# rwl/blu

Measured on AMD Instinct MI355X. Metric: factorize nnz/s + achieved HBM GB/s, 100k x 100k 10-nnz/col basis, higher is better.
Workload: dtype f64

## Files before the change

blu_amd/csrc/blu_dev.h:

```cpp
#pragma once
#include <hip/hip_runtime.h>
#include <stdint.h>
#include <hip/hip_cooperative_groups.h>
#include <rocprim/warp/warp_reduce.hpp>
#include <rocprim/warp/warp_scan.hpp>

#define BLU_WAVE 64

#ifndef BLU_DYN_SHARED
#define BLU_DYN_SHARED(T, name, bytes) extern __shared__ __attribute__((aligned(16))) T name[]
#endif
#ifdef BLU_PROFILE_FILLS
#define FILL_STAMP_BEGIN() long long fill_t0_ = (long long)__builtin_amdgcn_s_memtime()
#define FILL_STAMP(S, k)                                                 \
    do {                                                                 \
        if (threadIdx.x == 0) {                                          \
            const long long t_ = (long long)__builtin_amdgcn_s_memtime(); \
            (S)->prof[k] += t_ - fill_t0_;                               \
            fill_t0_ = t_;                                               \
        }                                                                \
    } while (0)
#else
#define FILL_STAMP_BEGIN() \
    do {                   \
// ... 33 lines not shown
    int bump_size;
    int cused, rused;
    int lused, uused;
    int need;
    int l_nz, u_nz;
    int fill_paths;
    long long matrix_nz;
    long long bump_nz;
    long long nsearch_pivot;
    long long factor_flops;
    long long nexpand;
    long long ngarbage;
    long long d3_hits;
    long long npivot_kind[6];
    long long nfast[4];
    long long nrun[2];
    double min_pivot, max_pivot;
    double onenorm, infnorm;
    double norm_l, norm_u, normest_l_inv, normest_u_inv, condest_l, condest_u, residual_test;
    long long prof[48];
    long long prof2[8];
};

#define DEVLU_SCALARS(X)                                                                               \
    X(int, m)                                                                                          \
    X(int, nzbias)                                                                      \
    X(int, maxsearch)                                                                                  \
    X(int, pad)                                                                                        \
    X(int, search_rows)                                                                                \
    X(int, no_fast)                    \
    X(int, skip_stats)              \
    X(double, droptol)                                                                                 \
    X(double, abstol)                                                                                  \
    X(double, reltol)                                                                                  \
    X(double, stretch)                                                                                 \
    X(long long, b_i_len)                                                                              \
// ... 515 lines not shown
```

blu_amd/csrc/blu_hip.hip:

```cpp
#include <hip/hip_runtime.h>

#include <algorithm>
#include <cmath>
#include <cstdio>
#include <cstdlib>
#include <cstring>
#include <string>
#include <vector>

#include "../../include/blu_hip.h"
#include "blu_dev.h"
#include "k_finish.hip"
#define BLU_NS pv_single
#define BLU_CFG_WAVE 0
#include "k_pivot.hip"
#undef BLU_NS
#undef BLU_CFG_WAVE
#define BLU_NS pv_wave
#define BLU_CFG_WAVE 1
#include "k_pivot.hip"
#undef BLU_NS
#undef BLU_CFG_WAVE
#define BLU_NS pv_wave2
#define BLU_CFG_WAVE 2
// ... 475 lines not shown
    case 51: return (double)s.npivot_kind[0];
    case 52: return (double)s.npivot_kind[1];
    case 53: return (double)s.npivot_kind[2];
    case 54: return (double)s.npivot_kind[3];
    case 55: return (double)s.npivot_kind[4];
    case 56: return (double)s.npivot_kind[5];
    case 110: case 111: case 116: case 117: return (double)s.nfast[key < 116 ? key - 110 : key - 114];
    case 112: return (double)s.cused;
    case 113: return (double)s.rused;
    case 114: return (double)h->D.carena_cap;
    case 115: return (double)h->D.lcap;
    case 120: return (double)h->last_pivot_regs;
    case 118: return (double)h->last_pivot_kernel;
    case 119: return (double)s.fill_paths;
    case 121: case 122: return (double)s.nrun[key - 121];
    case 131: case 132: case 133: case 134: case 135: case 136: case 137: case 138: return (double)s.prof2[key - 131];
    case 57: return (double)s.err_line;
    case 58: return (double)s.status;
    case 60: case 61: case 62: case 63: case 64: case 65: case 66: case 67: case 68: case 69: case 70: case 71: case 72: case 73: case 74: case 75:
    case 76: case 77: case 78: case 79: case 80: case 81: case 82: case 83:
    case 84: case 85: case 86: case 87: case 88: case 89: case 90: case 91:
    case 92: case 93: case 94: case 95: case 96: case 97: case 98: case 99: case 100: case 101: case 102: case 103: case 104: case 105: case 106: case 107:
        return (double)s.prof[key - 60];
    default: return NAN;
    }
}

extern "C" const char *blu_hip_last_error(const blu_hip *h) { return h ? h->err.c_str() : "null handle"; }
extern "C" const char *blu_hip_version(void)
{
#if defined(BLU_EWCHECK)
// ... 632 lines not shown
```

blu_amd/csrc/k_pivot.hip:

```cpp
#include "blu_dev.h"

namespace BLU_NS {

__shared__ int g_pivot_err;
__shared__ int g_pivot_err_line;
#undef DEV_CHECK
#define DEV_CHECK(S, cond)                               \
    do {                                                 \
        if (!(cond)) {                                   \
            set_error((S), ST_ERROR, __LINE__);          \
            g_pivot_err = 1;                             \
        }                                                \
    } while (0)

#if BLU_CFG_WAVE
#include "k_pivot_wave_types.h"
#else
#include "k_pivot_fast_types.h"
#endif

#ifdef BLU_PROFILE
__shared__ long long g_pstamp[56];
#define PROF_STAMP(k)                                                      \
    do {                                                                   \
// ... 14 lines not shown
#define PROF_WAIT() \
    do {            \
    } while (0)
#endif

struct alignas(16) Sm {
    Fast fa;
    struct alignas(16) {
        int pr, pc, exit_code, head_exit;
    };
    struct alignas(16) {
        int nzc, nzr, pcb, prb;
    };
#ifdef BLU_PROFILE
    long long prof[48];
    long long prof2[8];
#else
    long long prof[1];
#endif
#if !BLU_CFG_WAVE
    Fast fb;
    struct alignas(16) {
        int nx_pr, nx_pc, nx_nzr, nx_where;
    };
    int nx_prb, nx_pcb, nx_nsr;
    int mg;
    long long nrun[2];
#endif
    int rank, rankdef, min_colnz, min_rownz;
    int cused, rused, lused, uused;
    int need;
    int flag_small;
    int other_row, where, ncancel, nfill;
    int stop_at, need_search;
    double pivot, other_value;
    long long nsearch, flops, nexpand, d3;
    long long kinds[6];
    long long nfast[4];
    int sh[40];
    long long shl[20];
#if BLU_CFG_WAVE
    unsigned long long wmax[BLU_CFG_WAVE];
// ... 1057 lines not shown
        sm->uused = S->uused;
        sm->pr = S->pivot_row;
        sm->pc = S->pivot_col;
        sm->exit_code = 0;
        sm->need = 0;
        sm->nsearch = 0;
        sm->flops = 0;
        sm->nexpand = 0;
        sm->d3 = 0;
        sm->stop_at = stop_at;
        sm->fa.kind = 0;
        sm->fa.ewValid = 0;
        sm->fa.spOk = 0;
        for (int k = 0; k < 6; k++) sm->kinds[k] = 0;
        sm->mg = 0;
        sm->nrun[0] = sm->nrun[1] = 0;
#ifdef BLU_PROFILE
        for (int k = 0; k < 48; k++) sm->prof[k] = 0;
        for (int k = 0; k < 8; k++) sm->prof2[k] = 0;
        for (int k = 0; k < 56; k++) g_pstamp[k] = 0;
#endif
    }
    for (int k = tid; k < (int)blockDim.x; k += blockDim.x) sm->swork[k] = 0.0;
    if (tid < 16) sm->wmax[tid] = 0ull;
    for (int k = tid; k < 2 * KGMAX; k += blockDim.x) sm->fa.kg[0][k] = 0ull;
    if (tid == 0) {
        g_pivot_err = 0;
        g_pivot_err_line = 0;
    }
    mc_reset(D, mc, tid, (int)blockDim.x);
    __syncthreads();

#ifdef BLU_PROFILE
#define PROF_ADD(k, a, b)                                                                                           \
    do {                                                                                                            \
        const long long d_ = g_pstamp[a] - g_pstamp[b];                                                             \
        if (g_pstamp[b] >= g_pstamp[0] && d_ >= 0 && d_ < (1LL << 28)) sm->prof[k] += d_;                            \
    } while (0)
#define PROF_ADD2(k, a, b)                                                                                          \
    do {                                                                                                            \
        const long long d_ = g_pstamp[a] - g_pstamp[b];                                                             \
        if (g_pstamp[b] >= g_pstamp[0] && d_ >= 0 && d_ < (1LL << 28)) sm->prof2[k] += d_;                           \
    } while (0)
    auto prof_account = [&](int kind_done) {
        {
            const int kk = kind_done == 1 ? 1 : (kind_done == 2 ? 2 : 3);
            PROF_ADD(0, 1, 0);
            PROF_ADD(kk, 2, 1);
            sm->prof[3 + kk] += 1;
            if (kk == 1) {
                PROF_ADD(7, 3, 1);
                PROF_ADD(22, 6, 3);
                PROF_ADD(23, 24, 3);
                PROF_ADD(24, 25, 3);
                PROF_ADD(25, 26, 25);
                PROF_ADD(26, 27, 26);
                PROF_ADD(27, 28, 27);
                PROF_ADD(30, 30, 27);
                PROF_ADD(31, 31, 30);
                PROF_ADD(28, 29, 28);
                PROF_ADD(29, 2, 29);
                sm->prof[32] += sm->nzr - 1;
                sm->prof[33] += sm->nzc - 1;
                PROF_ADD(34, 33, 1);
                PROF_ADD(35, 34, 33);
                PROF_ADD(36, 35, 34);
                PROF_ADD(37, 36, 35);
                PROF_ADD(38, 37, 36);
                PROF_ADD(39, 38, 37);
                PROF_ADD(40, 3, 38);
                if (g_pstamp[44] > g_pstamp[1]) {
                    PROF_ADD(41, 41, 1);
                    PROF_ADD(42, 42, 41);
                    PROF_ADD(43, 43, 42);
                    PROF_ADD(44, 44, 43);
                    sm->prof[45] += 1;
                }
            }
            if (kk == 2) {
                PROF_ADD2(0, 1, 0);
                PROF_ADD2(1, 49, 48);
                PROF_ADD2(2, 50, 48);
                PROF_ADD2(3, 51, 48);
                PROF_ADD2(4, 2, 48);
                PROF_ADD2(5, 48, 1);
            }
            if (kk != 3) {
                PROF_ADD(8, 8, 0);
                PROF_ADD(9, 9, 8);
                PROF_ADD(10, 10, 9);
                PROF_ADD(11, 11, 10);
// ... 62 lines not shown
        if (pr < 0) {
            __syncthreads();
            if (tid == 0) {
                list_remove1(D.cflink, D.cblink, pc);
                mc->dirty = 1;
                sm->pc = -1;
                sm->rankdef++;
                sm->kinds[5]++;
            }
            __syncthreads();
            continue;
        }

        if (dA.z) break;
        PROF_STAMP(1);
        const int nz_col = dB.x;
        int nz_row = dB.y;
        const int kind = dC.x;
        bool ok = true;
        if (kind == 1) fast_small(D, sm, mc, pr, pc, nz_col, nz_row, ew_mcb, ew_fb);
        else if (kind == 2) {
            Fast *cs = &sm->fa;
            int wq = dC.y;
            for (;;) {
                fast_scol(D, sm, mc, cs, pr, pc, nz_row, wq, ew_mcb, ew_fb);
                if (!sm->mg) break;
#ifdef BLU_PROFILE
                PROF_STAMP(2);
                if (tid == 0) {
                    prof_account(2);
                    sm->prof2[6] += 1;
                    g_pstamp[0] = g_pstamp[1] = g_pstamp[2];
                }
#endif
                const int4 nx = *reinterpret_cast<const int4 *>(&sm->nx_pr);
                if (tid == (int)blockDim.x - 128) {
                    const int rank = sm->rank;
                    D.pinv[pr] = rank;
                    D.qinv[pc] = rank;
                    D.prow[rank] = pr;
                    D.pcol[rank] = pc;
                    sm->rank = rank + 1;
                    sm->nsearch += sm->nx_nsr;
                    sm->min_colnz = 1;
                    sm->nrun[0]++;
                    sm->nrun[1]++;
                }
                pr = nx.x;
                pc = nx.y;
                nz_row = nx.z;
                wq = nx.w;
                cs = cs == &sm->fa ? &sm->fb : &sm->fa;
#ifdef BLU_EWCHECK
                __syncthreads();
                if (w == 0) scol_setup_check(D, sm, mc, cs);
                __syncthreads();
#endif
            }
        } else {
            if (tid == 0) mc->dirty = 1;
            if (nz_row == 1) ok = pivot_singleton_row(D, sm);
            else if (nz_col == 1) ok = pivot_singleton_col(D, sm);
            else if (nz_col == 2) ok = pivot_doubleton_col(D, sm);
            else ok = pivot_general(D, sm, nz_col - 1 <= 64);
        }
        if (!ok) break;
        PROF_STAMP(2);
#ifdef BLU_PROFILE
        if (tid == 0) prof_account(kind);
#endif

        if (tid == 0) {
            const int rank = sm->rank;
            if (sm->flag_small && nz_row > 1) {
                for (int pos = D.ubeg[rank]; pos < D.ubeg[rank + 1]; pos++) {
                    const int j = D.uidx[pos];
                    if (D.colmax[j] == 0.0 || D.colmax[j] < D.abstol) {
                        remove_col_serial(D, sm, j);
                        mc->dirty = 1;
                    }
                }
            }
            sm->flops += (long long)(nz_col - 1) * (long long)(nz_row - 1);
            D.pinv[pr] = rank;
// ... 11 lines not shown
        S->rankdef = sm->rankdef;
        S->min_colnz = sm->min_colnz;
        S->min_rownz = sm->min_rownz;
        S->cused = sm->cused;
        S->rused = sm->rused;
        S->lused = sm->lused;
        S->uused = sm->uused;
        S->pivot_row = sm->pr;
        S->pivot_col = sm->pc;
        S->need = sm->need;
        S->nsearch_pivot += sm->nsearch;
        S->factor_flops += sm->flops;
        S->nexpand += sm->nexpand;
        S->d3_hits += sm->d3;
        for (int k = 0; k < 6; k++) S->npivot_kind[k] += sm->kinds[k];
        for (int k = 0; k < 2; k++) S->nrun[k] += sm->nrun[k];
#ifdef BLU_PROFILE
        for (int k = 0; k < 48; k++) S->prof[k] += sm->prof[k];
        for (int k = 0; k < 8; k++) S->prof2[k] += sm->prof2[k];
#endif
        if (sm->exit_code == ST_ERROR && g_pivot_err_line) set_error(S, ST_ERROR, g_pivot_err_line);
        if (S->status == ST_RUNNING) S->status = sm->exit_code;
    }
}

__global__ void __launch_bounds__(1024) k_pivot_loop(DevLU *Ds, int stop_at)
{
    __shared__ Sm smem;
    __shared__ Mc mcache;
    pivot_loop_body(Ds, stop_at, &smem, &mcache);
}
#endif

}
// ... 10 lines not shown
```

blu_amd/csrc/k_pivot_fast.hip:

```cpp

__device__ __forceinline__ unsigned hslot(int k, int bits) { return ((unsigned)k * 2654435761u) >> (32 - bits); }
__device__ __forceinline__ void probe_overrun(int line)
{
    g_pivot_err = 1;
    g_pivot_err_line = line;
}
__device__ __forceinline__ void hrow_insert(Fast *f, int k, int v)
{
    unsigned s = hslot(k, HROW_BITS);
    const unsigned long long want = ((unsigned long long)(unsigned)k << 32) | (unsigned)v;
    for (int n = 0; n < HROW; n++) {
        const unsigned long long old = atomicCAS(&f->hRow[s], ~0ull, want);
        if (old == ~0ull || (int)(old >> 32) == k) return;
        s = (s + 1) & (HROW - 1);
    }
    probe_overrun(__LINE__);
}
__device__ __forceinline__ int hrow_lookup(const Fast *f, int k)
{
    unsigned s = hslot(k, HROW_BITS);
    for (int n = 0; n < HROW; n++) {
        const unsigned long long x = f->hRow[s];
        if ((int)(x >> 32) == k) return (int)(x & 0xffffffffull);
        if (x == ~0ull) return 0;
// ... 892 lines not shown
        mk_pick(D, sm, 0, 0, nsr, true);
        return true;
    }
    const int r = mk_walk(D, sm, mc);
    PROF_STAMP(9);
    if (r == 3) return false;
    if (r != 0) return true;
    long long mcb;
    int fb;
    mk_stage(D, sm, mcb, fb);
    PROF_STAMP(10);
    mk_pick(D, sm, mcb, fb, fa->ncand, false);
    return true;
}

__device__ __forceinline__ void fast_col(const DevGP &D, Sm *sm, Mc *mc, int q, double *work, int idx_first, double val_first, int pr, int cnz1,
                                         double pivot)
{
    const int lane = lane_id();
    Scalars *S = D.s;
    Fast *fa = &sm->fa;
    const int j = fa->tJ[q], cb = fa->tB[q], cl = fa->tL[q], cap = fa->tC[q];

    int nkept = 0, where = -1, first_idx = 0;
    double xrj = 0.0, first_val = 0.0, cmxl = 0.0;
    int idx0 = 0, t0r = 0;
    double val0 = 0.0;
    bool keep0 = false;
    for (int c = 0; c < cl; c += 64) {
        const int e = c + lane;
        const bool v = e < cl;
        const int idx = c == 0 ? idx_first : (v ? D.cidx[cb + e] : 0);
        const double val = c == 0 ? val_first : (v ? D.cval[cb + e] : 0.0);
        const int mk = v ? hrow_lookup(fa, idx) : 0;
        const bool keep = v && mk == 0;
        if (v && mk > 0) work[mk - 1] = val;
// ... 101 lines not shown
        if (reloc) atomicAdd((unsigned long long *)&sm->nexpand, 1ull);
        if (mask >> 31) atomicAdd((unsigned long long *)&sm->d3, (unsigned long long)__popcll(mask >> 31));
        if (cmx == 0.0 || cmx < D.abstol) sm->flag_small = 1;
    }
}

__device__ __forceinline__ int hrow_lookup2(const Fast *f, int k)
{
    const unsigned s0 = hslot(k, HROW_BITS), s1 = (s0 + 1) & (HROW - 1);
    const unsigned long long x0 = f->hRow[s0], x1 = f->hRow[s1];
    const bool h0 = (int)(x0 >> 32) == k, e0 = x0 == ~0ull, h1 = (int)(x1 >> 32) == k, e1 = x1 == ~0ull;
    int r = h0 ? (int)(x0 & 0xffffffffull) : ((!e0 && h1) ? (int)(x1 & 0xffffffffull) : 0);
    if (!(h0 || e0 || h1 || e1)) r = hrow_lookup(f, k);
    return r;
}
__device__ __forceinline__ void fast_col_short(const DevGP &D, Sm *sm, Mc *mc, int q, double *work, int idx, double val, int pr, int cnz1,
                                               double pivot)
{
    const int lane = lane_id();
    Scalars *S = D.s;
    Fast *fa = &sm->fa;
    const int j = fa->tJ[q], cb = fa->tB[q], cl = fa->tL[q], cap = fa->tC[q];
    const bool v = lane < cl;
    const int mk = v ? hrow_lookup2(fa, idx) : 0;
    const bool keep = v && mk == 0;
    if (v && mk > 0) work[mk - 1] = val;
    const unsigned long long kb = __ballot(keep);
    const int t = wave_prefix_count(kb);
    const unsigned long long pb = __ballot(keep && idx == pr);
    DEV_CHECK(S, pb != 0ull);
    const int psrc = pb ? __ffsll((long long)pb) - 1 : 0;
    const int where = wave_bcast_i(t, psrc);
    const double xrj = wave_bcast_d(val, psrc);
    const int fsrc = kb ? __ffsll((long long)kb) - 1 : 0;
    const int first_idx = wave_bcast_i(idx, fsrc);
    const double first_val = wave_bcast_d(val, fsrc);
// ... 50 lines not shown
        fa->tNew[q] = newlen;
        if (q < 64) {
            fa->tB[q] = dst;
            fa->tMx[q] = cmx;
            mc->e1i[q] = -1;
        }
        fa->tX[q] = xrj;
        fa->tM[q] = mask;
        if (mask) fa->anycancel = 1;
        if (reloc) atomicAdd((unsigned long long *)&sm->nexpand, 1ull);
        if (mask >> 31) atomicAdd((unsigned long long *)&sm->d3, (unsigned long long)__popcll(mask >> 31));
        if (cmx == 0.0 || cmx < D.abstol) sm->flag_small = 1;
    }
}

__device__ __forceinline__ void fast_row(const DevGP &D, Sm *sm, int p, int j_first, int pc, int rnz1)
{
    const int lane = lane_id();
    Scalars *S = D.s;
    Fast *fa = &sm->fa;
    const int i = fa->pcI[p], rb = fa->prB[p], rl = fa->prL[p], cap = fa->prC[p];

    int nk = 0;
    bool found = false;
    int j0 = -1, t0r = 0;
    bool keep0 = false;
    for (int c = 0; c < rl; c += 64) {
        const int e = c + lane;
        const bool v = e < rl;
        const int j = c == 0 ? j_first : (v ? D.ridx[rb + e] : -1);
        const bool keep = v && !hcol_has(fa, j);
        if (__ballot(v && j == pc)) found = true;
        const unsigned long long kb = __ballot(keep);
        if (c == 0) {
            j0 = j;
// ... 35 lines not shown
        fa->rKept[p] = nk;
        fa->rDst[p] = dst;
        if (reloc) atomicAdd((unsigned long long *)&sm->nexpand, 1ull);
    }
}

__device__ __forceinline__ bool hcol_has2(const Fast *f, int k)
{
    const unsigned s0 = hslot(k, HCOL_BITS), s1 = (s0 + 1) & (HCOL - 1);
    const unsigned long long x0 = f->hCol[s0], x1 = f->hCol[s1];
    const bool h0 = (int)(x0 >> 32) == k, e0 = x0 == ~0ull, h1 = (int)(x1 >> 32) == k, e1 = x1 == ~0ull;
    bool r = h0 || (!e0 && h1);
    if (!(h0 || e0 || h1 || e1)) r = hcol_has(f, k);
    return r;
}
__device__ __forceinline__ void fast_row_short(const DevGP &D, Sm *sm, int p, int j, int pc, int rnz1)
{
    const int lane = lane_id();
    Scalars *S = D.s;
    Fast *fa = &sm->fa;
    const int i = fa->pcI[p], rb = fa->prB[p], rl = fa->prL[p], cap = fa->prC[p];
    const bool v = lane < rl;
    const bool keep = v && !hcol_has2(fa, j);
    DEV_CHECK(S, __ballot(v && j == pc) != 0ull);
    const unsigned long long kb = __ballot(keep);
    const int t0 = wave_prefix_count(kb);
    const int nk = __popcll(kb);
    const int need_max = nk + rnz1;
    const bool reloc = need_max > cap;
    int dst = rb, newcap = cap;
    if (reloc) {
        newcap = need_max + stretch_of(D.stretch, need_max) + D.pad;
        int nb = 0;
        if (lane == 0) nb = atomicAdd(&sm->rused, newcap);
        dst = __builtin_amdgcn_readfirstlane(nb);
    }
    if (keep) D.ridx[dst + t0] = j;
    for (int q = 1 + lane; q <= rnz1; q += 64) D.ridx[dst + nk + q - 1] = fa->tJ[q];
    if (lane == 0) {
        D.rbeg[i] = dst;
        D.rlen[i] = nk + rnz1;
        D.rcap[i] = newcap;
        fa->rNew[p] = nk + rnz1;
        fa->rKept[p] = nk;
        fa->rDst[p] = dst;
        if (reloc) atomicAdd((unsigned long long *)&sm->nexpand, 1ull);
    }
}

__device__ __forceinline__ void fast_fixrow(const DevGP &D, Sm *sm, int p)
{
    const int lane = lane_id();
    Fast *fa = &sm->fa;
    const int rnz1 = sm->nzr - 1;
    const int dst = fa->rDst[p], nk = fa->rKept[p];
    int na = 0;
    for (int c = 0; c < rnz1; c += 64) {
        const int q = 1 + c + lane;
        const bool ok = q <= rnz1 && ((fa->tM[q] >> (p - 1)) & 1ull) == 0;
        const unsigned long long kb = __ballot(ok);
        if (ok) D.ridx[dst + nk + na + wave_prefix_count(kb)] = fa->tJ[q];
        na += __popcll(kb);
    }
    if (lane == 0) {
        D.rlen[fa->pcI[p]] = nk + na;
        fa->rNew[p] = nk + na;
    }
}

// ... 18 lines not shown
        const bool k = v && fabs(x) > D.droptol;
        const unsigned long long kb = __ballot(k);
        if (k) {
            const int d = put + wave_prefix_count(kb);
            D.uidx[d] = fa->tJ[q];
            D.uval[d] = x;
        }
        put += __popcll(kb);
    }
    if (lane == 0) {
        D.ubeg[sm->rank + 1] = put;
        sm->uused = put;
    }
}

__device__ __forceinline__ void fast_write_l(const DevGP &D, Sm *sm)
{
    const int lane = lane_id();
    Fast *fa = &sm->fa;
    const int cnz1 = sm->nzc - 1;
    const double pivot = fa->pcV[0];
    int put = sm->lused;
    for (int c = 1; c <= cnz1; c += 64) {
        const int p = c + lane;
        const bool v = p <= cnz1;
        const double x = v ? fa->pcV[p] / pivot : 0.0;
        const bool k = v && fabs(x) > D.droptol;
        const unsigned long long kb = __ballot(k);
        if (k) {
            const int d = put + wave_prefix_count(kb);
            D.lidx[d] = fa->pcI[p];
            D.lval[d] = x;
        }
        put += __popcll(kb);
    }
    if (lane == 0) {
        D.lbeg[sm->rank + 1] = put;
        sm->lused = put;
    }
}

__device__ __forceinline__ void early_search(const DevGP &D, Sm *sm, Mc *mc, const Fast *cs, const int *elems, const int *keys, const int *begs, const double *maxs,
                                             int n, int ebase, long long &ew_mcb, int &ew_fb)
{
    const int lane = lane_id();
    const int m = D.m;
    Fast *fa = &sm->fa;
    const int K = D.maxsearch;
    if (D.search_rows || D.no_fast || K < 1 || K > KCMAX || m >= (1 << 27) || n >= 64) return;
    if (sm->flag_small || fa->anycancel) return;
    const int left = m - (sm->rank + 1) - sm->rankdef;
    if (left < 1) return;
    const int kq = lane < n ? keys[lane] : -1;
    if (__ballot(kq == 0)) return;
    int nsr = 0;

    {
        const int h1 = LinksC{D, mc}.fl(m + 1);
        const unsigned long long one = __ballot(kq == 1);
        int j = -1, cb = 0, fs = -1;
        double cmx = 0.0;
        if (h1 < m && !hcol_has(cs, h1)) {
            j = h1;
            cb = D.cbeg[j];
            cmx = D.colmax[j];
// ... 105 lines not shown
        }
        nz += 64;
    }
    if (bad || ncand < K || total > STGMAX) return;
    SPEC_STAT(1);
    if (lane == 0) {
        fa->cOff[ncand] = total;
        fa->ncand = ncand;
        fa->spLastNz = lastnz;
        fa->spOk = 1;
    }
    wave_mem_sync();
    PROF_STAMP_L0(42);
}

__device__ __forceinline__ bool spec_cond(const Sm *sm, const int *keys, int n)
{
    const int lane = lane_id();
    const Fast *fa = &sm->fa;
    if (!fa->spOk || sm->flag_small || fa->anycancel || n >= 64) return false;
    const int kq = lane < n ? keys[lane] : 0x7fffffff;
    return __ballot(kq <= 0) == 0ull;
}

__device__ __forceinline__ void spec_finish(const DevGP &D, Sm *sm, int n)
{
    const int lane = lane_id();
    Fast *fa = &sm->fa;
    const int ncand = fa->ncand;
    {
        const int lastnz = fa->spLastNz;
        const int key = lane < n ? fa->tNew[1 + lane] : 0x7fffffff;
        const unsigned long long inb = __ballot(key < lastnz);
        if (inb) {
            int uJ = 0, uNz = 0x7fffffff, uB = 0, uL = 0;
            double uMx = 0.0;
            if (lane < ncand) {
                uJ = fa->cJ[lane];
                uNz = fa->cNz[lane];
                uB = fa->cB[lane];
                uL = fa->cL[lane];
                uMx = fa->cMx[lane];
            }
            int ule = 0;
            for (int i = 0; i < ncand; i++) ule += fa->cNz[i] <= key;
            int before = 0, below = 0;
            unsigned long long mb = inb;
// ... 2 lines not shown
                mb &= mb - 1;
                const int kb = __builtin_amdgcn_readlane(key, b);
                before += (kb < key) || (kb == key && b < lane);
                below += kb < uNz;
            }
            const int posM = ule + before, posU = lane + below;
            wave_mem_sync();
            if (lane < ncand && posU < ncand) {
                fa->cJ[posU] = uJ;
                fa->cNz[posU] = uNz;
                fa->cB[posU] = uB;
                fa->cL[posU] = uL;
                fa->cMx[posU] = uMx;
            }
            if (((inb >> lane) & 1ull) && posM < ncand) {
                fa->cJ[posM] = fa->tJ[1 + lane];
                fa->cNz[posM] = key;
                fa->cB[posM] = fa->tB[1 + lane];
                fa->cL[posM] = key;
                fa->cMx[posM] = fa->tMx[1 + lane];
            }
            wave_mem_sync();
            if (lane == 0) {
                int off = 0;
                for (int i = 0; i < ncand; i++) {
                    fa->cOff[i] = off;
                    off += fa->cL[i];
                }
                fa->cOff[ncand] = off;
            }
            wave_mem_sync();
            SPEC_STAT(4);
        }
    }
    const int total = fa->cOff[ncand];
// ... 30 lines not shown
    PROF_WAIT();
    PROF_STAMP_L0(43);
    SPEC_STAT(2);
    const long long key = wave_min_ll(mcb != BIG ? mcb * 256LL + (long long)fb : BIG);
    if (key == BIG) return;
    SPEC_STAT(3);
    if (lane == 0) {
        fa->spKey = key;
        fa->ewNsr = ncand;
        fa->ewValid = 2;
    }
    wave_mem_sync();
    PROF_STAMP_L0(44);
}

__device__ __forceinline__ void fast_small(const DevGP &D, Sm *sm, Mc *mc, int pr, int pc, int nzc, int nzr, long long &ew_mcb, int &ew_fb)
{
    const int w = wave_id(), nw = num_waves(), lane = lane_id();
    const int m = D.m;
    Fast *fa = &sm->fa;
    const int cnz1 = nzc - 1, rnz1 = nzr - 1;
    const double pivot = fa->pcV[0];
    DEV_CHECK(D.s, pivot != 0.0);

    double *work = &sm->swork[w * 64];
    const int ntask = rnz1 + cnz1;
    PROF_STAMP(4);
    const bool split = nw >= 8 && rnz1 < 64;
    const int nwt = split ? nw - 1 : nw;
    const LinksC LC{D, mc};
    const bool early = split && !D.search_rows;
    if (split && w == nw - 1) {
        if (early) __builtin_amdgcn_s_setprio(3);
        const bool lnk = fa->tLnk != 0;
        wave_list_unlink_set(LC, fa->tJ + 1, rnz1, -1, InHCol{fa, 1, 0}, pc, lnk ? fa->tFl + 1 : nullptr, lnk ? fa->tBl + 1 : nullptr, -1);
// ... 33 lines not shown
                    li[u] = D.ridx[lb[u] + lane];
                }
            }
        }
#ifdef BLU_PROFILE
        if (w == 1 && base == 0) {
            PROF_STAMP_L0(33);
            PROF_WAIT();
            PROF_STAMP_L0(34);
        }
#endif
#pragma unroll
        for (int u = 0; u < 3; u++) {
            const int t = tt[u];
            if (t < rnz1) {
                if (ll[u] <= 64) fast_col_short(D, sm, mc, t + 1, work, li[u], lv[u], pr, cnz1, pivot);
                else fast_col(D, sm, mc, t + 1, work, li[u], lv[u], pr, cnz1, pivot);
            } else if (t < ntask) {
                if (ll[u] <= 64) fast_row_short(D, sm, t - rnz1 + 1, li[u], pc, rnz1);
                else fast_row(D, sm, t - rnz1 + 1, li[u], pc, rnz1);
            }
#ifdef BLU_PROFILE
            if (w == 1 && base == 0) PROF_STAMP_L0(35 + u);
#endif
        }
    }
#ifdef BLU_PROFILE
    if (w == 1) {
        PROF_WAIT();
        PROF_STAMP_L0(38);
    }
#endif
    PROF_STAMP(5);
    __syncthreads();
    PROF_STAMP(3);
    if (fa->anycancel) {
        for (int p = 1 + w; p <= cnz1; p += nw) fast_fixrow(D, sm, p);
        __syncthreads();
    }
    const bool spec = early && (w == 0 || w == nw - 1) && spec_cond(sm, fa->tNew + 1, rnz1);
    if (w == 0 && early && !spec) early_search(D, sm, mc, fa, fa->tJ + 1, fa->tNew + 1, fa->tB + 1, fa->tMx + 1, rnz1, 1, ew_mcb, ew_fb);
    if (w == nw - 1 && spec) spec_finish(D, sm, rnz1);
    if (w == (early ? 3 : 0)) {
        fast_write_u(D, sm, fa, 1, rnz1, -1);
        if (lane == 0) {
            D.colmax[pc] = fa->pcV[0];
            D.clen[pc] = 0;
            D.rlen[pr] = 0;
            sm->kinds[3]++;
        }
        PROF_STAMP_L0(6);
    }
    if (w == 1 % nw) {
        fast_write_l(D, sm);
        PROF_STAMP_L0(24);
    }
    if (w == 2 % nw) {
        PROF_STAMP_L0(25);
        const int mn = split ? wave_list_append_set(LC, m, fa->tJ + 1, fa->tNew + 1, rnz1, m + 2, fa->kg[0], mc->pFl + 1)
                             : wave_list_move_batch_set(LC, m, fa->tJ + 1, fa->tNew + 1, rnz1, InHCol{fa, 1, 0}, m + 2, pc, fa->kg[0]);
        if (lane == 0 && mn < sm->min_colnz) sm->min_colnz = mn;
        if (lane == 0) {
            mc->prevValid = split ? 1 : 0;
            mc->prevBase = 1;
        }
        PROF_WAIT();
        PROF_STAMP_L0(29);
    }
    if (D.search_rows && w == 3 % nw) {
        if (lane == 0) list_remove1(D.rflink, D.rblink, pr);
        wave_mem_sync();
        const int mn = wave_list_move_batch_set(LinksG{D.rflink, D.rblink}, m, fa->pcI + 1, fa->rNew + 1, cnz1, InHRow{fa}, m + 2, -1, fa->kg[1]);
        if (lane == 0 && mn < sm->min_rownz) sm->min_rownz = mn;
    }
    __syncthreads();
}

__device__ __forceinline__ bool scol_setup_next(const DevGP &D, Sm *sm, Mc *mc, Fast *nxt, int rl_cur)
{
    const int lane = lane_id();
    Fast *st = &sm->fa;
    if (st->ewValid != 1) return false;
    if (g_pivot_err || mc->dirty) return false;
    const int nrd = sm->rank + 1 + sm->rankdef;
    if (nrd >= D.m || (sm->stop_at >= 0 && nrd >= sm->stop_at)) return false;
    const int pc = st->cJ[0], pr = st->sI[0], prb = st->sB[0], nzr = st->sL[0];
    if (nzr < 2 || nzr >= 64) return false;
// ... 7 lines not shown
        const int tb = D.cbeg[jq0], tl = D.clen[jq0], tc = D.ccap[jq0];
        nxt->tJ[lane] = jq0;
        nxt->tB[lane] = tb;
        nxt->tL[lane] = tl;
        nxt->tC[lane] = tc;
        hcol_insert(nxt, jq0, lane);
    }
    if (lane == 0) {
        nxt->pcI[0] = pr;
        nxt->pcV[0] = st->sV[0];
        nxt->prB[0] = prb;
        nxt->prL[0] = nzr;
        nxt->prC[0] = st->sC[0];
        nxt->kind = 2;
        nxt->where = wpos;
        nxt->tLnk = 0;
        sm->nx_pr = pr;
        sm->nx_pc = pc;
        sm->nx_nzr = nzr;
        sm->nx_where = wpos;
        sm->nx_prb = prb;
        sm->nx_pcb = st->cB[0];
        sm->nx_nsr = st->ewNsr;
        st->ewValid = 0;
    }
    return true;
}

#ifdef BLU_EWCHECK
__device__ __forceinline__ void scol_setup_check(const DevGP &D, Sm *sm, Mc *mc, Fast *nxt)
{
    const int lane = lane_id();
    Fast *T = nxt;
    Fast *R = &sm->fa;
    if (nxt == R) {
        T = &sm->fb;
        T->tJ[lane] = R->tJ[lane];
        T->tB[lane] = R->tB[lane];
// ... 37 lines not shown
    if (lane == 0) {
        sm->pr = o_pr;
        sm->pc = o_pc;
        sm->pcb = o_pcb;
        sm->prb = o_prb;
        sm->nzc = o_nzc;
        sm->nzr = o_nzr;
        sm->exit_code = o_exit;
        sm->need = o_need;
        sm->min_colnz = o_minc;
        sm->nsearch = o_ns;
    }
    if (__ballot(!okc)) DEV_CHECK(D.s, false);
    wave_mem_sync();
}
#endif

__device__ __forceinline__ void fast_scol(const DevGP &D, Sm *sm, Mc *mc, Fast *fa, int pr, int pc, int rl, int wq, long long &ew_mcb, int &ew_fb)
{
    const int w = wave_id(), nw = num_waves(), lane = lane_id();
    const int m = D.m;
    Scalars *S = D.s;
    DEV_CHECK(S, fa->pcV[0] != 0.0 && fa->pcI[0] == pr);

    const bool split = nw >= 8 && rl < 64;
    const int nwt = split ? nw - 1 : nw;
    const LinksC LC{D, mc};
    if (split && w == nw - 1) {
        const bool lnk = fa->tLnk != 0;
        wave_list_unlink_set(LC, fa->tJ, rl, wq, InHCol{fa, 0, wq}, pc, lnk ? fa->tFl : nullptr, lnk ? fa->tBl : nullptr, wq);
// ... 126 lines not shown
```

Baseline: 1.384 million.

## Chain small-pivot fast path into next pivot via double-buffered setup

Extends the pivot-chaining loop so that the fast_small path, not just the singleton-column path, can prepare the next pivot directly in the alternate Fast buffer. After an early or speculative search it sets up the following pivot's column and row tables and hashes, checks arena capacity, and skips the kernel-loop round trip and separate search and setup. The fast helpers now take the Fast buffer as a parameter, and stats and profile counters are widened. This adds setup work on one wave and a risk of state mismatches, which a self-check build verifies.

```diff
diff --git a/blu_amd/csrc/blu_dev.h b/blu_amd/csrc/blu_dev.h
--- a/blu_amd/csrc/blu_dev.h
+++ b/blu_amd/csrc/blu_dev.h
@@ -71,12 +71,12 @@
     long long d3_hits;
     long long npivot_kind[6];
     long long nfast[4];
-    long long nrun[2];
+    long long nrun[4];
     double min_pivot, max_pivot;
     double onenorm, infnorm;
     double norm_l, norm_u, normest_l_inv, normest_u_inv, condest_l, condest_u, residual_test;
     long long prof[48];
-    long long prof2[8];
+    long long prof2[14];
 };
 
 #define DEVLU_SCALARS(X)                                                                               \
diff --git a/blu_amd/csrc/blu_hip.hip b/blu_amd/csrc/blu_hip.hip
--- a/blu_amd/csrc/blu_hip.hip
+++ b/blu_amd/csrc/blu_hip.hip
@@ -513,7 +513,10 @@
     case 118: return (double)h->last_pivot_kernel;
     case 119: return (double)s.fill_paths;
     case 121: case 122: return (double)s.nrun[key - 121];
-    case 131: case 132: case 133: case 134: case 135: case 136: case 137: case 138: return (double)s.prof2[key - 131];
+    case 123: return (double)s.nrun[2];
+    case 125: return (double)s.nrun[3];
+    case 131: case 132: case 133: case 134: case 135: case 136: case 137: case 138: case 139: case 140: case 141: case 142: case 143: case 144:
+        return (double)s.prof2[key - 131];
     case 57: return (double)s.err_line;
     case 58: return (double)s.status;
     case 60: case 61: case 62: case 63: case 64: case 65: case 66: case 67: case 68: case 69: case 70: case 71: case 72: case 73: case 74: case 75:
diff --git a/blu_amd/csrc/k_pivot.hip b/blu_amd/csrc/k_pivot.hip
--- a/blu_amd/csrc/k_pivot.hip
+++ b/blu_amd/csrc/k_pivot.hip
@@ -52,7 +52,7 @@
     };
 #ifdef BLU_PROFILE
     long long prof[48];
-    long long prof2[8];
+    long long prof2[14];
 #else
     long long prof[1];
 #endif
@@ -61,9 +61,13 @@
     struct alignas(16) {
         int nx_pr, nx_pc, nx_nzr, nx_where;
     };
-    int nx_prb, nx_pcb, nx_nsr;
+    struct alignas(16) {
+        int nx_nzc, nx_kind, nx_pcb, nx_prb;
+    };
+    int nx_nsr, nx_minc;
+    int nx_whole;
     int mg;
-    long long nrun[2];
+    long long nrun[4];
 #endif
     int rank, rankdef, min_colnz, min_rownz;
     int cused, rused, lused, uused;
@@ -1151,10 +1155,10 @@
         sm->fa.spOk = 0;
         for (int k = 0; k < 6; k++) sm->kinds[k] = 0;
         sm->mg = 0;
-        sm->nrun[0] = sm->nrun[1] = 0;
+        sm->nrun[0] = sm->nrun[1] = sm->nrun[2] = sm->nrun[3] = 0;
 #ifdef BLU_PROFILE
         for (int k = 0; k < 48; k++) sm->prof[k] = 0;
-        for (int k = 0; k < 8; k++) sm->prof2[k] = 0;
+        for (int k = 0; k < 14; k++) sm->prof2[k] = 0;
         for (int k = 0; k < 56; k++) g_pstamp[k] = 0;
 #endif
     }
@@ -1179,13 +1183,17 @@
         const long long d_ = g_pstamp[a] - g_pstamp[b];                                                             \
         if (g_pstamp[b] >= g_pstamp[0] && d_ >= 0 && d_ < (1LL << 28)) sm->prof2[k] += d_;                           \
     } while (0)
-    auto prof_account = [&](int kind_done) {
+    auto prof_account = [&](int kind_done, int nzc_done, int nzr_done) {
         {
             const int kk = kind_done == 1 ? 1 : (kind_done == 2 ? 2 : 3);
             PROF_ADD(0, 1, 0);
             PROF_ADD(kk, 2, 1);
             sm->prof[3 + kk] += 1;
             if (kk == 1) {
+                const int by = g_pstamp[1] == g_pstamp[0] ? 8 : 11;
+                PROF_ADD2(by, 2, 0);
+                PROF_ADD2(by + 1, 2, 3);
+                sm->prof2[by + 2] += 1;
                 PROF_ADD(7, 3, 1);
                 PROF_ADD(22, 6, 3);
                 PROF_ADD(23, 24, 3);
@@ -1197,8 +1205,8 @@
                 PROF_ADD(31, 31, 30);
                 PROF_ADD(28, 29, 28);
                 PROF_ADD(29, 2, 29);
-                sm->prof[32] += sm->nzr - 1;
-                sm->prof[33] += sm->nzc - 1;
+                sm->prof[32] += nzr_done - 1;
+                sm->prof[33] += nzc_done - 1;
                 PROF_ADD(34, 33, 1);
                 PROF_ADD(35, 34, 33);
                 PROF_ADD(36, 35, 34);
@@ -1212,6 +1220,11 @@
                     PROF_ADD(43, 43, 42);
                     PROF_ADD(44, 44, 43);
                     sm->prof[45] += 1;
+                }
+                if (g_pstamp[46] > g_pstamp[3]) {
+                    PROF_ADD(46, 45, 3);
+                    PROF_ADD(47, 46, 3);
+                    sm->prof2[7] += 1;
                 }
             }
             if (kk == 2) {
@@ -1304,46 +1317,55 @@
 
         if (dA.z) break;
         PROF_STAMP(1);
-        const int nz_col = dB.x;
+        int nz_col = dB.x;
         int nz_row = dB.y;
-        const int kind = dC.x;
+        int kind = dC.x;
         bool ok = true;
-        if (kind == 1) fast_small(D, sm, mc, pr, pc, nz_col, nz_row, ew_mcb, ew_fb);
-        else if (kind == 2) {
+        if (kind == 1 || kind == 2) {
             Fast *cs = &sm->fa;
             int wq = dC.y;
             for (;;) {
-                fast_scol(D, sm, mc, cs, pr, pc, nz_row, wq, ew_mcb, ew_fb);
+                if (kind == 1) fast_small(D, sm, mc, cs, pr, pc, nz_col, nz_row, ew_mcb, ew_fb);
+                else fast_scol(D, sm, mc, cs, pr, pc, nz_row, wq, ew_mcb, ew_fb);
                 if (!sm->mg) break;
+                const int4 nx = *reinterpret_cast<const int4 *>(&sm->nx_pr);
+                const int4 ny = *reinterpret_cast<const int4 *>(&sm->nx_nzc);
 #ifdef BLU_PROFILE
                 PROF_STAMP(2);
                 if (tid == 0) {
-                    prof_account(2);
-                    sm->prof2[6] += 1;
+                    prof_account(kind, nz_col, nz_row);
+                    if (ny.y == 2) sm->prof2[6] += 1;
                     g_pstamp[0] = g_pstamp[1] = g_pstamp[2];
                 }
 #endif
-                const int4 nx = *reinterpret_cast<const int4 *>(&sm->nx_pr);
-                if (tid == (int)blockDim.x - 128) {
+                if (tid == (int)blockDim.x - (ny.y == 1 ? 64 : 128)) {
                     const int rank = sm->rank;
                     D.pinv[pr] = rank;
                     D.qinv[pc] = rank;
                     D.prow[rank] = pr;
                     D.pcol[rank] = pc;
                     sm->rank = rank + 1;
+                    sm->flops += (long long)(nz_col - 1) * (long long)(nz_row - 1);
                     sm->nsearch += sm->nx_nsr;
-                    sm->min_colnz = 1;
-                    sm->nrun[0]++;
-                    sm->nrun[1]++;
+                    sm->min_colnz = sm->nx_minc;
+                    if (!sm->nx_whole) sm->nrun[0]++;
+                    if (kind == 2 && ny.y == 2) sm->nrun[1]++;
+                    if (ny.y == 1) sm->nrun[2]++;
+                    if (kind == 1 && ny.y == 2) sm->nrun[3]++;
                 }
                 pr = nx.x;
                 pc = nx.y;
                 nz_row = nx.z;
                 wq = nx.w;
+                nz_col = ny.x;
+                kind = ny.y;
                 cs = cs == &sm->fa ? &sm->fb : &sm->fa;
 #ifdef BLU_EWCHECK
                 __syncthreads();
-                if (w == 0) scol_setup_check(D, sm, mc, cs);
+                if (w == 0) {
+                    if (sm->nx_whole) small_setup_check(D, sm, mc, cs);
+                    else scol_setup_check(D, sm, mc, cs);
+                }
                 __syncthreads();
 #endif
             }
@@ -1357,7 +1379,7 @@
         if (!ok) break;
         PROF_STAMP(2);
 #ifdef BLU_PROFILE
-        if (tid == 0) prof_account(kind);
+        if (tid == 0) prof_account(kind, nz_col, nz_row);
 #endif
 
         if (tid == 0) {
@@ -1399,10 +1421,10 @@
         S->nexpand += sm->nexpand;
         S->d3_hits += sm->d3;
         for (int k = 0; k < 6; k++) S->npivot_kind[k] += sm->kinds[k];
-        for (int k = 0; k < 2; k++) S->nrun[k] += sm->nrun[k];
+        for (int k = 0; k < 4; k++) S->nrun[k] += sm->nrun[k];
 #ifdef BLU_PROFILE
         for (int k = 0; k < 48; k++) S->prof[k] += sm->prof[k];
-        for (int k = 0; k < 8; k++) S->prof2[k] += sm->prof2[k];
+        for (int k = 0; k < 14; k++) S->prof2[k] += sm->prof2[k];
 #endif
         if (sm->exit_code == ST_ERROR && g_pivot_err_line) set_error(S, ST_ERROR, g_pivot_err_line);
         if (S->status == ST_RUNNING) S->status = sm->exit_code;
diff --git a/blu_amd/csrc/k_pivot_fast.hip b/blu_amd/csrc/k_pivot_fast.hip
--- a/blu_amd/csrc/k_pivot_fast.hip
+++ b/blu_amd/csrc/k_pivot_fast.hip
@@ -930,12 +930,11 @@
     return true;
 }
 
-__device__ __forceinline__ void fast_col(const DevGP &D, Sm *sm, Mc *mc, int q, double *work, int idx_first, double val_first, int pr, int cnz1,
-                                         double pivot)
+__device__ __forceinline__ void fast_col(const DevGP &D, Sm *sm, Mc *mc, Fast *fa, int q, double *work, int idx_first, double val_first, int pr,
+                                         int cnz1, double pivot)
 {
     const int lane = lane_id();
     Scalars *S = D.s;
-    Fast *fa = &sm->fa;
     const int j = fa->tJ[q], cb = fa->tB[q], cl = fa->tL[q], cap = fa->tC[q];
 
     int nkept = 0, where = -1, first_idx = 0;
@@ -1067,12 +1066,11 @@
     if (!(h0 || e0 || h1 || e1)) r = hrow_lookup(f, k);
     return r;
 }
-__device__ __forceinline__ void fast_col_short(const DevGP &D, Sm *sm, Mc *mc, int q, double *work, int idx, double val, int pr, int cnz1,
-                                               double pivot)
+__device__ __forceinline__ void fast_col_short(const DevGP &D, Sm *sm, Mc *mc, Fast *fa, int q, double *work, int idx, double val, int pr,
+                                               int cnz1, double pivot)
 {
     const int lane = lane_id();
     Scalars *S = D.s;
-    Fast *fa = &sm->fa;
     const int j = fa->tJ[q], cb = fa->tB[q], cl = fa->tL[q], cap = fa->tC[q];
     const bool v = lane < cl;
     const int mk = v ? hrow_lookup2(fa, idx) : 0;
@@ -1153,11 +1151,10 @@
     }
 }
 
-__device__ __forceinline__ void fast_row(const DevGP &D, Sm *sm, int p, int j_first, int pc, int rnz1)
+__device__ __forceinline__ void fast_row(const DevGP &D, Sm *sm, Fast *fa, int p, int j_first, int pc, int rnz1)
 {
     const int lane = lane_id();
     Scalars *S = D.s;
-    Fast *fa = &sm->fa;
     const int i = fa->pcI[p], rb = fa->prB[p], rl = fa->prL[p], cap = fa->prC[p];
 
     int nk = 0;
@@ -1223,11 +1220,10 @@
     if (!(h0 || e0 || h1 || e1)) r = hcol_has(f, k);
     return r;
 }
-__device__ __forceinline__ void fast_row_short(const DevGP &D, Sm *sm, int p, int j, int pc, int rnz1)
+__device__ __forceinline__ void fast_row_short(const DevGP &D, Sm *sm, Fast *fa, int p, int j, int pc, int rnz1)
 {
     const int lane = lane_id();
     Scalars *S = D.s;
-    Fast *fa = &sm->fa;
     const int i = fa->pcI[p], rb = fa->prB[p], rl = fa->prL[p], cap = fa->prC[p];
     const bool v = lane < rl;
     const bool keep = v && !hcol_has2(fa, j);
@@ -1257,11 +1253,9 @@
     }
 }
 
-__device__ __forceinline__ void fast_fixrow(const DevGP &D, Sm *sm, int p)
+__device__ __forceinline__ void fast_fixrow(const DevGP &D, Fast *fa, int p, int rnz1)
 {
     const int lane = lane_id();
-    Fast *fa = &sm->fa;
-    const int rnz1 = sm->nzr - 1;
     const int dst = fa->rDst[p], nk = fa->rKept[p];
     int na = 0;
     for (int c = 0; c < rnz1; c += 64) {
@@ -1310,11 +1304,9 @@
     }
 }
 
-__device__ __forceinline__ void fast_write_l(const DevGP &D, Sm *sm)
+__device__ __forceinline__ void fast_write_l(const DevGP &D, Sm *sm, const Fast *fa, int cnz1)
 {
     const int lane = lane_id();
-    Fast *fa = &sm->fa;
-    const int cnz1 = sm->nzc - 1;
     const double pivot = fa->pcV[0];
     int put = sm->lused;
     for (int c = 1; c <= cnz1; c += 64) {
@@ -1344,7 +1336,7 @@
     Fast *fa = &sm->fa;
     const int K = D.maxsearch;
     if (D.search_rows || D.no_fast || K < 1 || K > KCMAX || m >= (1 << 27) || n >= 64) return;
-    if (sm->flag_small || fa->anycancel) return;
+    if (sm->flag_small || cs->anycancel) return;
     const int left = m - (sm->rank + 1) - sm->rankdef;
     if (left < 1) return;
     const int kq = lane < n ? keys[lane] : -1;
@@ -1480,23 +1472,22 @@
     PROF_STAMP_L0(42);
 }
 
-__device__ __forceinline__ bool spec_cond(const Sm *sm, const int *keys, int n)
+__device__ __forceinline__ bool spec_cond(const Sm *sm, const Fast *cs, const int *keys, int n)
 {
     const int lane = lane_id();
-    const Fast *fa = &sm->fa;
-    if (!fa->spOk || sm->flag_small || fa->anycancel || n >= 64) return false;
+    if (!sm->fa.spOk || sm->flag_small || cs->anycancel || n >= 64) return false;
     const int kq = lane < n ? keys[lane] : 0x7fffffff;
     return __ballot(kq <= 0) == 0ull;
 }
 
-__device__ __forceinline__ void spec_finish(const DevGP &D, Sm *sm, int n)
+__device__ __forceinline__ void spec_finish(const DevGP &D, Sm *sm, const Fast *cs, int n)
 {
     const int lane = lane_id();
     Fast *fa = &sm->fa;
     const int ncand = fa->ncand;
     {
         const int lastnz = fa->spLastNz;
-        const int key = lane < n ? fa->tNew[1 + lane] : 0x7fffffff;
+        const int key = lane < n ? cs->tNew[1 + lane] : 0x7fffffff;
         const unsigned long long inb = __ballot(key < lastnz);
         if (inb) {
             int uJ = 0, uNz = 0x7fffffff, uB = 0, uL = 0;
@@ -1529,11 +1520,11 @@
                 fa->cMx[posU] = uMx;
             }
             if (((inb >> lane) & 1ull) && posM < ncand) {
-                fa->cJ[posM] = fa->tJ[1 + lane];
+                fa->cJ[posM] = cs->tJ[1 + lane];
                 fa->cNz[posM] = key;
-                fa->cB[posM] = fa->tB[1 + lane];
+                fa->cB[posM] = cs->tB[1 + lane];
                 fa->cL[posM] = key;
-                fa->cMx[posM] = fa->tMx[1 + lane];
+                fa->cMx[posM] = cs->tMx[1 + lane];
             }
             wave_mem_sync();
             if (lane == 0) {
@@ -1594,11 +1585,12 @@
     PROF_STAMP_L0(44);
 }
 
-__device__ __forceinline__ void fast_small(const DevGP &D, Sm *sm, Mc *mc, int pr, int pc, int nzc, int nzr, long long &ew_mcb, int &ew_fb)
+__device__ __forceinline__ bool scol_setup_next(const DevGP &D, Sm *sm, Mc *mc, Fast *nxt, int rl_cur);
+__device__ __forceinline__ bool small_setup_next(const DevGP &D, Sm *sm, Mc *mc, Fast *nxt, int cnz1_cur, int rnz1_cur);
+__device__ __forceinline__ void fast_small(const DevGP &D, Sm *sm, Mc *mc, Fast *fa, int pr, int pc, int nzc, int nzr, long long &ew_mcb, int &ew_fb)
 {
     const int w = wave_id(), nw = num_waves(), lane = lane_id();
     const int m = D.m;
-    Fast *fa = &sm->fa;
     const int cnz1 = nzc - 1, rnz1 = nzr - 1;
     const double pivot = fa->pcV[0];
     DEV_CHECK(D.s, pivot != 0.0);
@@ -1662,11 +1654,11 @@
         for (int u = 0; u < 3; u++) {
             const int t = tt[u];
             if (t < rnz1) {
-                if (ll[u] <= 64) fast_col_short(D, sm, mc, t + 1, work, li[u], lv[u], pr, cnz1, pivot);
-                else fast_col(D, sm, mc, t + 1, work, li[u], lv[u], pr, cnz1, pivot);
+                if (ll[u] <= 64) fast_col_short(D, sm, mc, fa, t + 1, work, li[u], lv[u], pr, cnz1, pivot);
+                else fast_col(D, sm, mc, fa, t + 1, work, li[u], lv[u], pr, cnz1, pivot);
             } else if (t < ntask) {
-                if (ll[u] <= 64) fast_row_short(D, sm, t - rnz1 + 1, li[u], pc, rnz1);
-                else fast_row(D, sm, t - rnz1 + 1, li[u], pc, rnz1);
+                if (ll[u] <= 64) fast_row_short(D, sm, fa, t - rnz1 + 1, li[u], pc, rnz1);
+                else fast_row(D, sm, fa, t - rnz1 + 1, li[u], pc, rnz1);
             }
 #ifdef BLU_PROFILE
             if (w == 1 && base == 0) PROF_STAMP_L0(35 + u);
@@ -1683,12 +1675,26 @@
     __syncthreads();
     PROF_STAMP(3);
     if (fa->anycancel) {
-        for (int p = 1 + w; p <= cnz1; p += nw) fast_fixrow(D, sm, p);
+        for (int p = 1 + w; p <= cnz1; p += nw) fast_fixrow(D, fa, p, rnz1);
         __syncthreads();
     }
-    const bool spec = early && (w == 0 || w == nw - 1) && spec_cond(sm, fa->tNew + 1, rnz1);
-    if (w == 0 && early && !spec) early_search(D, sm, mc, fa, fa->tJ + 1, fa->tNew + 1, fa->tB + 1, fa->tMx + 1, rnz1, 1, ew_mcb, ew_fb);
-    if (w == nw - 1 && spec) spec_finish(D, sm, rnz1);
+    const bool spec = early && (w == 0 || w == nw - 1) && spec_cond(sm, fa, fa->tNew + 1, rnz1);
+    Fast *other = fa == &sm->fa ? &sm->fb : &sm->fa;
+    if (w == 0 && !spec) {
+        bool merged = false;
+        if (early) {
+            early_search(D, sm, mc, fa, fa->tJ + 1, fa->tNew + 1, fa->tB + 1, fa->tMx + 1, rnz1, 1, ew_mcb, ew_fb);
+            merged = scol_setup_next(D, sm, mc, other, rnz1 + 1);
+        }
+        if (lane == 0) sm->mg = merged ? 1 : 0;
+    }
+    if (w == nw - 1 && spec) {
+        spec_finish(D, sm, fa, rnz1);
+        PROF_STAMP_L0(45);
+        const bool merged = small_setup_next(D, sm, mc, other, cnz1, rnz1);
+        if (lane == 0) sm->mg = merged ? 1 : 0;
+        PROF_STAMP_L0(46);
+    }
     if (w == (early ? 3 : 0)) {
         fast_write_u(D, sm, fa, 1, rnz1, -1);
         if (lane == 0) {
@@ -1700,16 +1706,16 @@
         PROF_STAMP_L0(6);
     }
     if (w == 1 % nw) {
-        fast_write_l(D, sm);
+        fast_write_l(D, sm, fa, cnz1);
         PROF_STAMP_L0(24);
     }
     if (w == 2 % nw) {
         PROF_STAMP_L0(25);
-        const int mn = split ? wave_list_append_set(LC, m, fa->tJ + 1, fa->tNew + 1, rnz1, m + 2, fa->kg[0], mc->pFl + 1)
-                             : wave_list_move_batch_set(LC, m, fa->tJ + 1, fa->tNew + 1, rnz1, InHCol{fa, 1, 0}, m + 2, pc, fa->kg[0]);
+        const int mn = split ? wave_list_append_set(LC, m, fa->tJ + 1, fa->tNew + 1, rnz1, m + 2, sm->fa.kg[0], mc->pFl + 1)
+                             : wave_list_move_batch_set(LC, m, fa->tJ + 1, fa->tNew + 1, rnz1, InHCol{fa, 1, 0}, m + 2, pc, sm->fa.kg[0]);
         if (lane == 0 && mn < sm->min_colnz) sm->min_colnz = mn;
         if (lane == 0) {
-            mc->prevValid = split ? 1 : 0;
+            mc->prevValid = split && fa == &sm->fa ? 1 : 0;
             mc->prevBase = 1;
         }
         PROF_WAIT();
@@ -1718,7 +1724,7 @@
     if (D.search_rows && w == 3 % nw) {
         if (lane == 0) list_remove1(D.rflink, D.rblink, pr);
         wave_mem_sync();
-        const int mn = wave_list_move_batch_set(LinksG{D.rflink, D.rblink}, m, fa->pcI + 1, fa->rNew + 1, cnz1, InHRow{fa}, m + 2, -1, fa->kg[1]);
+        const int mn = wave_list_move_batch_set(LinksG{D.rflink, D.rblink}, m, fa->pcI + 1, fa->rNew + 1, cnz1, InHRow{fa}, m + 2, -1, sm->fa.kg[1]);
         if (lane == 0 && mn < sm->min_rownz) sm->min_rownz = mn;
     }
     __syncthreads();
@@ -1756,14 +1762,114 @@
         nxt->prC[0] = st->sC[0];
         nxt->kind = 2;
         nxt->where = wpos;
+        nxt->anycancel = 0;
         nxt->tLnk = 0;
         sm->nx_pr = pr;
         sm->nx_pc = pc;
         sm->nx_nzr = nzr;
         sm->nx_where = wpos;
+        sm->nx_nzc = 1;
+        sm->nx_kind = 2;
         sm->nx_prb = prb;
         sm->nx_pcb = st->cB[0];
         sm->nx_nsr = st->ewNsr;
+        sm->nx_minc = 1;
+        sm->nx_whole = 0;
+        st->ewValid = 0;
+    }
+    return true;
+}
+
+__device__ __forceinline__ bool small_setup_next(const DevGP &D, Sm *sm, Mc *mc, Fast *nxt, int cnz1_cur, int rnz1_cur)
+{
+    const int lane = lane_id();
+    Fast *st = &sm->fa;
+    if (st->ewValid != 2) return false;
+    if (g_pivot_err || mc->dirty) return false;
+    const int nrd = sm->rank + 1 + sm->rankdef;
+    if (nrd >= D.m || (sm->stop_at >= 0 && nrd >= sm->stop_at)) return false;
+    const int ncand = st->ncand;
+    const int off1 = ncand > 1 ? st->cOff[1] : 0x7fffffff, off2 = ncand > 2 ? st->cOff[2] : 0x7fffffff,
+              off3 = ncand > 3 ? st->cOff[3] : 0x7fffffff;
+    const int fsel = (int)(st->spKey & 255LL);
+    const int csel = (fsel >= off1) + (fsel >= off2) + (fsel >= off3);
+    const int coff = st->cOff[csel];
+    const int pc = st->cJ[csel], pr = st->sI[fsel];
+    const int nzc = st->cL[csel], pcb = st->cB[csel], where = fsel - coff;
+    const int nzr = st->sL[fsel], prb = st->sB[fsel];
+    int kind = 0;
+    if (nzr >= 2 && nzr <= 64) {
+        if (nzc == 1) kind = 2;
+        else if (nzc >= 3 && nzc <= 64) kind = 1;
+    }
+    if (kind == 0) return false;
+    if ((long long)sm->lused + cnz1_cur + (nzc - 1) > (long long)D.lcap || (long long)sm->uused + rnz1_cur + (nzr - 1) > (long long)D.ucap) return false;
+    const int jq0 = lane < nzr ? D.ridx[prb + lane] : -1;
+    if (kind == 1) {
+        for (int s = lane; s < HROW; s += 64) nxt->hRow[s] = ~0ull;
+    }
+    for (int s = lane; s < HCOL; s += 64) nxt->hCol[s] = ~0ull;
+    int hr_idx0 = 0, hr_slot0 = 0, hr_len0 = 0;
+    if (lane < nzc) {
+        const int slot = (lane == where) ? 0 : (lane == 0 ? where : lane);
+        const int idx = st->sI[coff + lane], rlv = st->sL[coff + lane];
+        nxt->pcI[slot] = idx;
+        nxt->pcV[slot] = st->sV[coff + lane];
+        nxt->prB[slot] = st->sB[coff + lane];
+        nxt->prL[slot] = rlv;
+        nxt->prC[slot] = st->sC[coff + lane];
+        hr_slot0 = slot;
+        hr_idx0 = idx;
+        hr_len0 = rlv;
+    }
+    const unsigned long long hb = __ballot(jq0 == pc);
+    if (!hb) return false;
+    const int wpos = __ffsll((long long)hb) - 1;
+    int tb = 0, tl = 0, tc = 0;
+    if (lane < nzr) {
+        tb = D.cbeg[jq0];
+        tl = D.clen[jq0];
+        tc = D.ccap[jq0];
+    }
+    int gc = 0, gr = 0;
+    if (kind == 1 && hr_slot0 >= 1) {
+        hrow_insert(nxt, hr_idx0, hr_slot0);
+        const int n = hr_len0 + nzr - 1;
+        gr = n + stretch_of(D.stretch, n) + D.pad;
+    }
+    if (lane < nzr) {
+        const int slot = kind == 1 ? ((lane == wpos) ? 0 : (lane == 0 ? wpos : lane)) : lane;
+        nxt->tJ[slot] = jq0;
+        nxt->tB[slot] = tb;
+        nxt->tL[slot] = tl;
+        nxt->tC[slot] = tc;
+        hcol_insert(nxt, jq0, slot);
+        if (kind == 1 && lane != wpos) {
+            const int n = tl + nzc - 1;
+            gc = n + stretch_of(D.stretch, n) + D.pad;
+        }
+    }
+    if (kind == 1) {
+        const long long both = wave_sum_ll(((long long)gc << 32) | (long long)(unsigned)gr);
+        if ((long long)sm->cused + (both >> 32) > (long long)D.carena_cap || (long long)sm->rused + (both & 0xffffffffLL) > (long long)D.rarena_cap)
+            return false;
+    }
+    if (lane == 0) {
+        nxt->kind = kind;
+        nxt->where = wpos;
+        nxt->anycancel = 0;
+        nxt->tLnk = 0;
+        sm->nx_pr = pr;
+        sm->nx_pc = pc;
+        sm->nx_nzr = nzr;
+        sm->nx_where = wpos;
+        sm->nx_nzc = nzc;
+        sm->nx_kind = kind;
+        sm->nx_prb = prb;
+        sm->nx_pcb = pcb;
+        sm->nx_nsr = st->ewNsr;
+        sm->nx_minc = st->cNz[0];
+        sm->nx_whole = 1;
         st->ewValid = 0;
     }
     return true;
@@ -1831,6 +1937,99 @@
     if (__ballot(!okc)) DEV_CHECK(D.s, false);
     wave_mem_sync();
 }
+
+__device__ __forceinline__ void small_setup_check(const DevGP &D, Sm *sm, Mc *mc, Fast *nxt)
+{
+    const int lane = lane_id();
+    Fast *T = nxt;
+    Fast *R = &sm->fa;
+    const int n = sm->nx_nzr, nc = sm->nx_nzc, knd = sm->nx_kind;
+    if (nxt == R) {
+        T = &sm->fb;
+        T->tJ[lane] = R->tJ[lane];
+        T->tB[lane] = R->tB[lane];
+        T->tL[lane] = R->tL[lane];
+        T->tC[lane] = R->tC[lane];
+        T->pcI[lane] = R->pcI[lane];
+        T->pcV[lane] = R->pcV[lane];
+        T->prB[lane] = R->prB[lane];
+        T->prL[lane] = R->prL[lane];
+        T->prC[lane] = R->prC[lane];
+        for (int s = lane; s < HCOL; s += 64) T->hCol[s] = R->hCol[s];
+        for (int s = lane; s < HROW; s += 64) T->hRow[s] = R->hRow[s];
+        if (lane == 0) {
+            T->kind = R->kind;
+            T->where = R->where;
+            T->anycancel = R->anycancel;
+        }
+    }
+    wave_mem_sync();
+    const int o_pr = sm->pr, o_pc = sm->pc, o_pcb = sm->pcb, o_prb = sm->prb, o_nzc = sm->nzc, o_nzr = sm->nzr;
+    const int o_exit = sm->exit_code, o_need = sm->need, o_minc = sm->min_colnz;
+    const long long o_ns = sm->nsearch;
+    wave_mem_sync();
+    if (lane == 0) sm->min_colnz = 1;
+    wave_mem_sync();
+    int nsr2 = 0;
+    bool okc = true;
+    if (mk_express(D, sm, mc, nsr2)) {
+        mk_pick(D, sm, 0, 0, nsr2, true);
+    } else if (mk_walk(D, sm, mc) == 0) {
+        long long mcb2;
+        int fb2;
+        mk_stage(D, sm, mcb2, fb2);
+        nsr2 = R->ncand;
+        mk_pick(D, sm, mcb2, fb2, nsr2, false);
+    } else {
+        okc = false;
+    }
+    wave_mem_sync();
+    if (okc) {
+        okc = sm->pr == sm->nx_pr && sm->pc == sm->nx_pc && sm->nzr == n && sm->nzc == nc && sm->prb == sm->nx_prb && sm->pcb == sm->nx_pcb &&
+              nsr2 == sm->nx_nsr && sm->exit_code == o_exit && sm->min_colnz == o_minc && sm->min_colnz == sm->nx_minc && R->kind == knd &&
+              T->kind == knd && R->where == T->where && R->where == sm->nx_where && R->anycancel == 0 && T->anycancel == 0;
+        if (okc && lane < n) {
+            const int j = T->tJ[lane];
+            okc = R->tJ[lane] == j && R->tB[lane] == T->tB[lane] && R->tL[lane] == T->tL[lane] && R->tC[lane] == T->tC[lane] &&
+                  hcol_slot(R, j) == lane && hcol_slot(T, j) == lane;
+        }
+        if (okc && lane < nc) {
+            const int i = T->pcI[lane];
+            okc = R->pcI[lane] == i && R->pcV[lane] == T->pcV[lane] && R->prB[lane] == T->prB[lane] && R->prL[lane] == T->prL[lane] &&
+                  R->prC[lane] == T->prC[lane];
+            if (okc && knd == 1 && lane >= 1) okc = hrow_lookup(R, i) == lane && hrow_lookup(T, i) == lane;
+        }
+        int cntR = 0, cntT = 0;
+        for (int s = lane; s < HCOL; s += 64) {
+            cntR += __popcll(__ballot(R->hCol[s] != ~0ull));
+            cntT += __popcll(__ballot(T->hCol[s] != ~0ull));
+        }
+        okc = okc && cntR == n && cntT == n;
+        if (knd == 1) {
+            cntR = cntT = 0;
+            for (int s = lane; s < HROW; s += 64) {
+                cntR += __popcll(__ballot(R->hRow[s] != ~0ull));
+                cntT += __popcll(__ballot(T->hRow[s] != ~0ull));
+            }
+            okc = okc && cntR == nc - 1 && cntT == nc - 1;
+        }
+    }
+    wave_mem_sync();
+    if (lane == 0) {
+        sm->pr = o_pr;
+        sm->pc = o_pc;
+        sm->pcb = o_pcb;
+        sm->prb = o_prb;
+        sm->nzc = o_nzc;
+        sm->nzr = o_nzr;
+        sm->exit_code = o_exit;
+        sm->need = o_need;
+        sm->min_colnz = o_minc;
+        sm->nsearch = o_ns;
+    }
+    if (__ballot(!okc)) DEV_CHECK(D.s, false);
+    wave_mem_sync();
+}
 #endif
 
 __device__ __forceinline__ void fast_scol(const DevGP &D, Sm *sm, Mc *mc, Fast *fa, int pr, int pc, int rl, int wq, long long &ew_mcb, int &ew_fb)
```

New measurement: 1.419 million, median of 6. 1.03x the previous value.
